# tongdaxu/VQ-VAE-from-Gaussian-VAE

Measured on AMD Instinct MI355X. Metric: images/sec encode+quantize+decode, 256x256, codebook 2^16, higher is better.
Workload: dtype f32

## Files before the change

vq-vae-from-gaussian-vae_amd/csrc/gq_conv3.h:

```cpp
#pragma once
#include <type_traits>

#include "gq_common.h"
#include "gq_epilogue.h"
#include "gq_stats.h"
#include "gq_wino_gemm.h"

namespace gqhip {

constexpr int kC3TH = 8, kC3TW = 32;
constexpr int kC3PH = kC3TH + 2, kC3PW = kC3TW + 2;
constexpr int kC3Pix = kC3PH * kC3PW;
constexpr int kC3RS = 48;
constexpr int kC3Plane = kC3PH * kC3RS * 32;
constexpr int kC3Buf = 2 * kC3Plane;
constexpr int kC3Pieces = kC3Pix * 4;
constexpr int kC3Loads = (kC3Pieces + 255) / 256;

__device__ __forceinline__ int conv3_lds_off(int R, int x, int half) {
  return (R * kC3RS + x) * 32 + 16 * (half ^ ((x >> 3) & 1));
}

struct Conv3Params {
  const _Float16 *Xs;
  const _Float16 *Wf;
  const float *bias;
  const float *res;
  float *y;
  int64_t *stats;
  int H, W, nch, cpg;
  int cout, nnb;
  int tiles_x, tiles_y;
  long ntiles;
  long tiles_per_xcd;
  float mscale;
};

struct Conv3Tile {
  long b;
  int y0, x0, nb;
};
__device__ __forceinline__ bool conv3_tile(const Conv3Params &p, Conv3Tile &t, long vb = blockIdx.x) {
  const long k = vb >> 3;
  t.nb = (int)(k % p.nnb);
  const long tile = (long)(vb & 7) * p.tiles_per_xcd + k / p.nnb;
  if (tile >= p.ntiles) return false;
  const int tx = (int)(tile % p.tiles_x);
  const long t2 = tile / p.tiles_x;
  t.b = t2 / p.tiles_y;
  t.y0 = (int)(t2 % p.tiles_y) * kC3TH;
  t.x0 = tx * kC3TW;
  return true;
}

__device__ __forceinline__ void conv3_tap(const unsigned char *A, int dy, const f16x8 (&bq)[4], f32x16 (&acc)[4][2]) {
#pragma unroll
  for (int rr = 0; rr < 4; ++rr) {
#if defined(GQHIP_ABL) && (GQHIP_ABL & 256)
    const f16x8 ah = *reinterpret_cast<const f16x8 *>(A + dy * kC3RS * 32);
    const f16x8 al = ah;
#else
    const f16x8 ah = *reinterpret_cast<const f16x8 *>(A + (rr + dy) * kC3RS * 32);
    const f16x8 al = *reinterpret_cast<const f16x8 *>(A + (rr + dy) * kC3RS * 32 + kC3Plane);
#endif
#pragma unroll
    for (int j = 0; j < 2; ++j) {
      acc[rr][j] = __builtin_amdgcn_mfma_f32_32x32x16_f16(ah, bq[2 * j], acc[rr][j], 0, 0, 0);
      acc[rr][j] = __builtin_amdgcn_mfma_f32_32x32x16_f16(ah, bq[2 * j + 1], acc[rr][j], 0, 0, 0);
      acc[rr][j] = __builtin_amdgcn_mfma_f32_32x32x16_f16(al, bq[2 * j], acc[rr][j], 0, 0, 0);
    }
  }
}

template <int COUT, int RR>
__device__ __forceinline__ void conv3_epilogue(const Conv3Params &p, const Conv3Tile &t, const f32x16 (&acc)[RR][2], unsigned char *sA,
                                               int64_t *red, int wave, int wm, int wn) {
  constexpr int cout = COUT;
  const int lane = __lane_id(), tid = wave * 64 + lane;
  const int n = wn * 64 + 4 * (lane & 15);
  float *stage = reinterpret_cast<float *>(sA + wave * kEpiWaveBytes);
  f32x4 pb = {0.f, 0.f, 0.f, 0.f};
  if (p.bias) {
#pragma unroll
    for (int e = 0; e < 4; ++e) pb[e] = p.bias[t.nb * 128 + n + e];
  }
  const long o = ((t.b * p.H + t.y0 + RR * wm) * p.W + t.x0 + (lane >> 4)) * cout + t.nb * 128 + n;
  const long slice = (long)p.W * cout;
  StatPartial st;
  if (!p.stats) {
    if (p.res) epi_store<3, false>(acc, stage, lane, p.y, p.res, o, slice, 4 * cout, p.mscale, pb, st);
    else epi_store<2, false>(acc, stage, lane, p.y, nullptr, o, slice, 4 * cout, p.mscale, pb, st);
    return;
  }
  if constexpr (RR == 4) {
    if (p.res) epi_store<3, true>(acc, stage, lane, p.y, p.res, o, slice, 4 * cout, p.mscale, pb, st);
    else epi_store<2, true>(acc, stage, lane, p.y, nullptr, o, slice, 4 * cout, p.mscale, pb, st);
    stat_partial_flush(red + kStatWords * (n / p.cpg), st);
  } else {
    __shared__ double part[2 * 64 * 4];
    double *mine = part + (wn * 64 + lane) * 4;
    if (wm == 0) {
      if (p.res) epi_store<3, true>(acc, stage, lane, p.y, p.res, o, slice, 4 * cout, p.mscale, pb, st);
      else epi_store<2, true>(acc, stage, lane, p.y, nullptr, o, slice, 4 * cout, p.mscale, pb, st);
      mine[0] = st.v0; mine[1] = st.s; mine[2] = st.ss; mine[3] = (double)st.n;
    }
    __syncthreads();
    if (wm == 1) {
      st.v0 = mine[0]; st.s = mine[1]; st.ss = mine[2]; st.n = (int)mine[3];
      if (p.res) epi_store<3, true>(acc, stage, lane, p.y, p.res, o, slice, 4 * cout, p.mscale, pb, st);
      else epi_store<2, true>(acc, stage, lane, p.y, nullptr, o, slice, 4 * cout, p.mscale, pb, st);
      stat_partial_flush(red + kStatWords * (n / p.cpg), st);
    }
  }
  __syncthreads();
  const int gpb = 128 / p.cpg, groups = cout / p.cpg;
  if (tid < kStatWords * gpb) stat_flush_word(p.stats + kStatWords * (t.b * groups + t.nb * gpb) + tid, red[tid]);
}

#define GQ_C3_ZERO_ACC(acc)                                                                                         \
  _Pragma("unroll") for (int rr = 0; rr < 4; ++rr) _Pragma("unroll") for (int j = 0; j < 2; ++j) acc[rr][j] =       \
      f32x16{0.f, 0.f, 0.f, 0.f, 0.f, 0.f, 0.f, 0.f, 0.f, 0.f, 0.f, 0.f, 0.f, 0.f, 0.f, 0.f}

struct Conv3GnParams {
  Conv3Params c;
  const float *x;
  const float *gamma, *beta, *pre_bias;
  const int64_t *stats_in;
  int cin, cpg_in;
  double eps;
  float scale;
};

#ifdef GQHIP_CLOCK_STAMPS
__device__ unsigned long long g_c3_stamps[4 * 8192];
#endif
template <int SILU, int COUT>
__global__ __launch_bounds__(256, 2) void conv3x3_gn_f16x3_kernel(const Conv3GnParams pp) {
  typedef _Float16 f16x4 __attribute__((ext_vector_type(4)));
  const Conv3Params &p = pp.c;
  __shared__ __attribute__((aligned(16))) unsigned char sA[2 * kC3Buf];
  __shared__ int64_t red[kStatWords * 32];
  __shared__ __attribute__((aligned(16))) float sAff[2][512];
  const int tid = threadIdx.x, lane = tid & 63, wave = __builtin_amdgcn_readfirstlane(tid >> 6);
  const int c = lane & 31, h = lane >> 5, wm = wave >> 1, wn = wave & 1;
#ifdef GQHIP_CLOCK_STAMPS
  const unsigned long long st_r0 = __builtin_amdgcn_s_memrealtime();
#endif
  Conv3Tile t;
  if (!conv3_tile(p, t)) return;
  const int H = p.H, W = p.W, cin = pp.cin;
  red[tid] = 0;
  {
    const int groups = cin / pp.cpg_in;
    const double n = (double)pp.cpg_in * (double)H * (double)W;
    for (int ch = tid; ch < cin; ch += 256) {
      const int g = ch / pp.cpg_in;
      double st_s, st_ss;
      stat_load(pp.stats_in + kStatWords * (t.b * groups + g), st_s, st_ss);
      const double mean = st_s / n;
      double var = st_ss / n - mean * mean;
      var = var > 0.0 ? var : 0.0;
      const double rstd = 1.0 / sqrt(var + pp.eps);
      const double pbk = pp.pre_bias ? (double)pp.pre_bias[ch] : 0.0;
      sAff[0][ch] = (float)(rstd * (double)pp.gamma[ch]);
      sAff[1][ch] = (float)((double)pp.beta[ch] + (pbk - mean) * rstd * (double)pp.gamma[ch]);
    }
  }
  const int w = tid & 3, qs = tid >> 2;
  int goff[kC3Loads];
  unsigned inb = 0;
#pragma unroll
  for (int i = 0; i < kC3Loads; ++i) {
    int q = qs + 64 * i;
    q = q < kC3Pix ? q : kC3Pix - 1;
    const int R = q / kC3PW, px = q % kC3PW;
    const int gy = t.y0 - 1 + R, gx = t.x0 - 1 + px;
    const bool in = gy >= 0 && gy < H && gx >= 0 && gx < W;
    const int cy = gy < 0 ? 0 : (gy >= H ? H - 1 : gy), cx = gx < 0 ? 0 : (gx >= W ? W - 1 : gx);
    goff[i] = (cy * W + cx) * cin + 4 * w;
    inb |= (unsigned)(in ? 1 : 0) << i;
  }
  const float *xb = pp.x + t.b * (long)H * W * cin;
  f32x4 st[3];
  auto issue = [&](int i, int chunk) { st[i % 3] = *reinterpret_cast<const f32x4 *>(xb + goff[i] + chunk * 16); };
  auto convert = [&](int i, int chunk, int buf) {
    const int q = qs + 64 * i;
    if (q >= kC3Pix) return;
    const f32x4 a4 = *reinterpret_cast<const f32x4 *>(&sAff[0][chunk * 16 + 4 * w]);
    const f32x4 sh4 = *reinterpret_cast<const f32x4 *>(&sAff[1][chunk * 16 + 4 * w]);
    const f32x4 v = gn_act<SILU>(st[i % 3], a4, sh4) * (((inb >> i) & 1) ? pp.scale : 0.f);
    f16x4 hi, lo;
#pragma unroll
    for (int e = 0; e < 4; ++e) {
      hi[e] = (_Float16)v[e];
      lo[e] = (_Float16)(v[e] - (float)hi[e]);
    }
    const int off = buf * kC3Buf + conv3_lds_off(q / kC3PW, q % kC3PW, w >> 1) + 8 * (w & 1);
    *reinterpret_cast<f16x4 *>(&sA[off]) = hi;
    *reinterpret_cast<f16x4 *>(&sA[off + kC3Plane]) = lo;
  };

  f32x16 acc[4][2];
  GQ_C3_ZERO_ACC(acc);
  int aoff[3];
#pragma unroll
  for (int dx = 0; dx < 3; ++dx) aoff[dx] = conv3_lds_off(4 * wm, c + dx, h);
  const unsigned char *wbase = reinterpret_cast<const unsigned char *>(p.Wf) + (4 * t.nb + 2 * wn) * 128 * 16;
  const int wl = lane * 16;
  const long wstep = (long)p.nnb * (512 * 16);
  f16x8 bs[3][4];
  auto load_b = [&](int ks, f16x8 (&dst)[4]) {
    const unsigned char *s = wbase + ks * wstep;
#pragma unroll
    for (int k = 0; k < 4; ++k) dst[k] = *reinterpret_cast<const f16x8 *>(s + k * 1024 + wl);
  };
  const int nks = p.nch * 9;
// ... 188 lines not shown
      for (int i = 0; i < NI; ++i) convert(i, nbuf);
    }
    __builtin_amdgcn_sched_barrier(0);
    __syncthreads();
  }
  if constexpr (SPLIT != 0) {
    const int C = p.cout / 3, col = t.nb * 128, third = col / C;
    const int n = wn * 64 + 4 * (lane & 15), cc = col - third * C + n;
    const long L = (long)p.H * 32, tok = (long)(t.y0 + RR * wm) * 32 + (lane >> 4);
    f32x4 pb = {0.f, 0.f, 0.f, 0.f};
    if (p.bias) {
#pragma unroll
      for (int e = 0; e < 4; ++e) pb[e] = p.bias[col + n + e];
    }
    float *stage = reinterpret_cast<float *>(sA + wave * kEpiWaveBytes);
    if (third < 2) {
      _Float16 *dst = third == 0 ? pp.Q3 : pp.K3;
      epi_store_split(acc, stage, lane, dst, (t.b * L + tok) * 3 * C + cc, 32L * 3 * C, 4L * 3 * C, (long)C, third == 0, p.mscale,
                      pb, pp.sq);
    } else {
      epi_store_split(acc, stage, lane, pp.V3, (t.b * 3 * L + tok) * C + cc, 32L * C, 4L * C, L * C, false, p.mscale, pb, pp.sv);
    }
  } else {
    conv3_epilogue<COUT>(p, t, acc, sA, red, wave, wm, wn);
  }
}

struct Conv3S2Params {
  Conv3Params c;
  const float *x;
  const float *scales_dev;
  float scale;
  int cin, Hin, Win;
};

template <int COUT>
__global__ __launch_bounds__(256, 2) void conv3x3s2_f16x3_kernel(const Conv3S2Params pp) {
  typedef _Float16 f16x4 __attribute__((ext_vector_type(4)));
  Conv3Params p = pp.c;
  __shared__ __attribute__((aligned(16))) unsigned char sA[2 * kC3Buf];
  __shared__ int64_t red[kStatWords * 32];
  const int tid = threadIdx.x, lane = tid & 63, wave = __builtin_amdgcn_readfirstlane(tid >> 6);
  const int c = lane & 31, h = lane >> 5, wm = wave >> 1, wn = wave & 1;
  Conv3Tile t;
  if (!conv3_tile(p, t)) return;
  red[tid] = 0;
  const float scale = pp.scales_dev ? pp.scales_dev[0] : pp.scale;
  if (pp.scales_dev) p.mscale = pp.scales_dev[1];
  const int cin = pp.cin, nch = p.nch, Hin = pp.Hin, Win = pp.Win;
  constexpr int PR = kC3TH + 1, PC = kC3TW + 1, NP = 5;
  const int w = tid & 3, qs = tid >> 2;
  const float *xb = pp.x + t.b * (long)Hin * Win * cin + 4 * w;
  int goff[NP], loff[NP];
  unsigned inb = 0;
  auto setup_phase = [&](int a, int b) {
    inb = 0;
#pragma unroll
    for (int i = 0; i < NP; ++i) {
      const int q = qs + 64 * i;
      const int qq = q < PR * PC ? q : PR * PC - 1;
      const int R = qq / PC, X = qq % PC;
      const int gy = 2 * (t.y0 + R) + a, gx = 2 * (t.x0 + X) + b;
      const bool in = gy < Hin && gx < Win;
      const int cy = gy < Hin ? gy : Hin - 1, cx = gx < Win ? gx : Win - 1;
      goff[i] = (cy * Win + cx) * cin;
      loff[i] = q < PR * PC ? conv3_lds_off(R, X, w >> 1) + 8 * (w & 1) : -1;
      inb |= (unsigned)(in ? 1 : 0) << i;
    }
  };
  f32x4 st[NP];
  auto issue = [&](int chunk) {
#pragma unroll
    for (int i = 0; i < NP; ++i) st[i] = *reinterpret_cast<const f32x4 *>(xb + goff[i] + chunk * 16);
  };
  auto commit = [&](int buf) {
#pragma unroll
    for (int i = 0; i < NP; ++i) {
      if (loff[i] < 0) continue;
      const f32x4 v = st[i] * (((inb >> i) & 1) ? scale : 0.f);
      f16x4 hi, lo;
#pragma unroll
      for (int e = 0; e < 4; ++e) {
        hi[e] = (_Float16)v[e];
        lo[e] = (_Float16)(v[e] - (float)hi[e]);
      }
      unsigned char *d = sA + buf * kC3Buf + loff[i];
      *reinterpret_cast<f16x4 *>(d) = hi;
      *reinterpret_cast<f16x4 *>(d + kC3Plane) = lo;
    }
  };
  f32x16 acc[4][2];
  GQ_C3_ZERO_ACC(acc);
  int aoff[2];
#pragma unroll
  for (int dx = 0; dx < 2; ++dx) aoff[dx] = conv3_lds_off(4 * wm, c + dx, h);
  const unsigned char *wbase = reinterpret_cast<const unsigned char *>(p.Wf) + (4 * t.nb + 2 * wn) * 128 * 16;
  const int wl = lane * 16;
  const long wstep = (long)p.nnb * (512 * 16);
  f16x8 bq[4], bn[4];
  auto load_b = [&](int ks, f16x8 (&dst)[4]) {
    const unsigned char *s = wbase + ks * wstep;
#pragma unroll
    for (int k = 0; k < 4; ++k) dst[k] = *reinterpret_cast<const f16x8 *>(s + k * 1024 + wl);
  };
  const int nks = 9 * nch;
  int ks = 0, unit = 0;
  load_b(0, bq);
  setup_phase(0, 0);
  issue(0);
  commit(0);
  __syncthreads();
  auto run_unit = [&](auto nt_tag, auto a_tag, auto b_tag, int chunk) {
    constexpr int NT = decltype(nt_tag)::value, PA = decltype(a_tag)::value, PB = decltype(b_tag)::value;
    const bool last_chunk = chunk + 1 >= nch;
    const bool more = !(last_chunk && PA == 1 && PB == 1);
    if (more) {
      if (last_chunk) setup_phase(PB == 1 ? 1 : PA, PB == 1 ? 0 : 1);
      issue(last_chunk ? 0 : chunk + 1);
    }
    const unsigned char *A = sA + (unit & 1) * kC3Buf;
#pragma unroll
    for (int ti = 0; ti < NT; ++ti) {
      const int ddy = (PA == 0 && PB == 0) ? ti / 2 : (PA == 0 && PB == 1) ? ti : 0;
      const int ddx = (PA == 0 && PB == 0) ? ti % 2 : (PA == 1 && PB == 0) ? ti : 0;
      load_b(ks + 1 < nks ? ks + 1 : ks, bn);
      conv3_tap(A + aoff[ddx], ddy, bq, acc);
#pragma unroll
      for (int k = 0; k < 4; ++k) bq[k] = bn[k];
      ++ks;
      __builtin_amdgcn_sched_barrier(0);
    }
    if (more) commit((unit + 1) & 1);
    ++unit;
    __syncthreads();
  };
  using I0 = std::integral_constant<int, 0>; using I1 = std::integral_constant<int, 1>;
  using I2 = std::integral_constant<int, 2>; using I4 = std::integral_constant<int, 4>;
  for (int chunk = 0; chunk < nch; ++chunk) run_unit(I4{}, I0{}, I0{}, chunk);
  for (int chunk = 0; chunk < nch; ++chunk) run_unit(I2{}, I0{}, I1{}, chunk);
  for (int chunk = 0; chunk < nch; ++chunk) run_unit(I2{}, I1{}, I0{}, chunk);
  for (int chunk = 0; chunk < nch; ++chunk) run_unit(I1{}, I1{}, I1{}, chunk);
  conv3_epilogue<COUT>(p, t, acc, sA, red, wave, wm, wn);
}

struct Upconv2Params {
  Conv3Params c;
  const float *x;
  const float *scales_dev;
  float scale;
  int cin;
};

template <int COUT>
__global__ __launch_bounds__(256, 2) void upconv2x_f16x3_kernel(const Upconv2Params pp) {
  typedef _Float16 f16x4 __attribute__((ext_vector_type(4)));
  Conv3Params p = pp.c;
  __shared__ __attribute__((aligned(16))) unsigned char sA[2 * kC3Buf];
  __shared__ int64_t red[kStatWords * 32];
  const int tid = threadIdx.x, lane = tid & 63, wave = __builtin_amdgcn_readfirstlane(tid >> 6);
  const int c = lane & 31, h = lane >> 5, wm = wave >> 1, wn = wave & 1;
  Conv3Tile t;
  if (!conv3_tile(p, t)) return;
  const int pa = (int)blockIdx.y >> 1, pb = (int)blockIdx.y & 1;
  red[tid] = 0;
  const float scale = pp.scales_dev ? pp.scales_dev[0] : pp.scale;
  if (pp.scales_dev) p.mscale = pp.scales_dev[1];
  const int cin = pp.cin, nch = p.nch, H = p.H, W = p.W;
  constexpr int PR = kC3TH + 1, PC = kC3TW + 1, NP = 5;
  const int w = tid & 3, qs = tid >> 2;
  const float *xb = pp.x + t.b * (long)H * W * cin + 4 * w;
  int goff[NP], loff[NP];
  unsigned inb = 0;
#pragma unroll
  for (int i = 0; i < NP; ++i) {
    const int q = qs + 64 * i;
    const int qq = q < PR * PC ? q : PR * PC - 1;
    const int R = qq / PC, X = qq % PC;
    const int gy = t.y0 + R + pa - 1, gx = t.x0 + X + pb - 1;
    const bool in = gy >= 0 && gy < H && gx >= 0 && gx < W;
    const int cy = gy < 0 ? 0 : (gy >= H ? H - 1 : gy), cx = gx < 0 ? 0 : (gx >= W ? W - 1 : gx);
    goff[i] = (cy * W + cx) * cin;
    loff[i] = q < PR * PC ? conv3_lds_off(R, X, w >> 1) + 8 * (w & 1) : -1;
    inb |= (unsigned)(in ? 1 : 0) << i;
  }
  f32x4 st[NP];
  auto issue = [&](int chunk) {
#pragma unroll
    for (int i = 0; i < NP; ++i) st[i] = *reinterpret_cast<const f32x4 *>(xb + goff[i] + chunk * 16);
  };
  auto commit = [&](int buf) {
#pragma unroll
    for (int i = 0; i < NP; ++i) {
      if (loff[i] < 0) continue;
      const f32x4 v = st[i] * (((inb >> i) & 1) ? scale : 0.f);
      f16x4 hi, lo;
#pragma unroll
      for (int e = 0; e < 4; ++e) {
        hi[e] = (_Float16)v[e];
        lo[e] = (_Float16)(v[e] - (float)hi[e]);
      }
      unsigned char *d = sA + buf * kC3Buf + loff[i];
      *reinterpret_cast<f16x4 *>(d) = hi;
      *reinterpret_cast<f16x4 *>(d + kC3Plane) = lo;
    }
  };
  f32x16 acc[4][2];
  GQ_C3_ZERO_ACC(acc);
  int aoff[2];
#pragma unroll
  for (int dx = 0; dx < 2; ++dx) aoff[dx] = conv3_lds_off(4 * wm, c + dx, h);
  const long wstep = (long)p.nnb * (512 * 16);
  const int nks = 4 * nch;
  const unsigned char *wbase = reinterpret_cast<const unsigned char *>(p.Wf) + (long)blockIdx.y * nks * wstep +
                               (4 * t.nb + 2 * wn) * 128 * 16;
  const int wl = lane * 16;
  f16x8 b0[4], b1[4], b2[4];
  auto load_b = [&](int ks, f16x8 (&dst)[4]) {
    const unsigned char *s = wbase + (long)(ks < nks ? ks : nks - 1) * wstep;
#pragma unroll
    for (int k = 0; k < 4; ++k) dst[k] = *reinterpret_cast<const f16x8 *>(s + k * 1024 + wl);
  };
  load_b(0, b0);
  load_b(1, b1);
  issue(0);
  commit(0);
  __syncthreads();
  int ks = 0;
  for (int chunk = 0; chunk < nch; ++chunk) {
    const bool more = chunk + 1 < nch;
    if (more) issue(chunk + 1);
    const unsigned char *A = sA + (chunk & 1) * kC3Buf;
#pragma unroll
    for (int ti = 0; ti < 4; ++ti) {
      load_b(ks + 2, b2);
      conv3_tap(A + aoff[ti & 1], ti >> 1, b0, acc);
#pragma unroll
      for (int k = 0; k < 4; ++k) {
        b0[k] = b1[k];
        b1[k] = b2[k];
      }
      ++ks;
      __builtin_amdgcn_sched_barrier(0);
    }
    if (more) commit((chunk + 1) & 1);
    __syncthreads();
  }
  constexpr int cout = COUT;
  const int n = wn * 64 + 4 * (lane & 15);
  f32x4 bias4 = {0.f, 0.f, 0.f, 0.f};
  if (p.bias) {
#pragma unroll
    for (int e = 0; e < 4; ++e) bias4[e] = p.bias[t.nb * 128 + n + e];
  }
  float *stage = reinterpret_cast<float *>(sA + wave * kEpiWaveBytes);
  const long W2 = 2L * W;
  const long o = ((t.b * 2L * H + 2 * (t.y0 + 4 * wm) + pa) * W2 + 2 * (t.x0 + (lane >> 4)) + pb) * cout + t.nb * 128 + n;
  StatPartial sp;
  if (!p.stats) {
    epi_store<1, false>(acc, stage, lane, p.y, nullptr, o, 2 * W2 * cout, 8 * cout, p.mscale, bias4, sp);
    return;
  }
  epi_store<1, true>(acc, stage, lane, p.y, nullptr, o, 2 * W2 * cout, 8 * cout, p.mscale, bias4, sp);
  stat_partial_flush(red + kStatWords * (n / p.cpg), sp);
  __syncthreads();
  const int gpb = 128 / p.cpg, groups = cout / p.cpg;
  if (tid < kStatWords * gpb) stat_flush_word(p.stats + kStatWords * (t.b * groups + t.nb * gpb) + tid, red[tid]);
}

template <int SILU, int COUT>
__global__ __launch_bounds__(256) void conv3x3_gn_small_kernel(const float *__restrict__ x, const float *__restrict__ gamma,
                                                               const float *__restrict__ beta,
                                                               const float *__restrict__ pre_bias,
                                                               const int64_t *__restrict__ stats, const float *__restrict__ w,
                                                               const float *__restrict__ bias, float *__restrict__ y, int H,
                                                               int W, int C, int cpg, double eps) {
  constexpr int PW = 18, PS = 36;
  __shared__ __attribute__((aligned(16))) float sX[PW * PW * PS];
  __shared__ __attribute__((aligned(16))) float sAff[2][512];
  const int tid = threadIdx.x, tx = tid & 15, ty = tid >> 4;
  const int tiles_x = W / 16, tiles_y = H / 16;
  const int txb = blockIdx.x % tiles_x, tyb = (blockIdx.x / tiles_x) % tiles_y;
  const long b = blockIdx.x / (tiles_x * tiles_y);
  const int y0 = tyb * 16, x0 = txb * 16;
  {
    const int groups = C / cpg;
    const double n = (double)cpg * (double)H * (double)W;
    for (int ch = tid; ch < C; ch += 256) {
      const int g = ch / cpg;
      double st_s, st_ss;
      stat_load(stats + kStatWords * (b * groups + g), st_s, st_ss);
      const double mean = st_s / n;
      double var = st_ss / n - mean * mean;
      var = var > 0.0 ? var : 0.0;
      const double rstd = 1.0 / sqrt(var + eps);
      const double pbk = pre_bias ? (double)pre_bias[ch] : 0.0;
      sAff[0][ch] = (float)(rstd * (double)gamma[ch]);
      sAff[1][ch] = (float)((double)beta[ch] + (pbk - mean) * rstd * (double)gamma[ch]);
    }
  }
  float acc[COUT];
#pragma unroll
  for (int co = 0; co < COUT; ++co) acc[co] = bias ? bias[co] : 0.f;
  const float *xb = x + b * (long)H * W * C;
  __syncthreads();
  for (int c0 = 0; c0 < C; c0 += 32) {
    for (int i = tid; i < PW * PW * 8; i += 256) {
      const int px = i >> 3, q = i & 7;
      const int R = px / PW, X = px % PW;
      const int gy = y0 - 1 + R, gx = x0 - 1 + X;
      const bool in = gy >= 0 && gy < H && gx >= 0 && gx < W;
      const int cy = gy < 0 ? 0 : (gy >= H ? H - 1 : gy), cx = gx < 0 ? 0 : (gx >= W ? W - 1 : gx);
      const f32x4 v = *reinterpret_cast<const f32x4 *>(xb + ((long)cy * W + cx) * C + c0 + 4 * q);
      const f32x4 a4 = *reinterpret_cast<const f32x4 *>(&sAff[0][c0 + 4 * q]);
      const f32x4 sh4 = *reinterpret_cast<const f32x4 *>(&sAff[1][c0 + 4 * q]);
      *reinterpret_cast<f32x4 *>(&sX[px * PS + 4 * q]) = gn_act<SILU>(v, a4, sh4) * (in ? 1.f : 0.f);
    }
    __syncthreads();
#pragma unroll
    for (int tap = 0; tap < 9; ++tap) {
      const float *s = &sX[((ty + tap / 3) * PW + tx + tap % 3) * PS];
#pragma unroll
      for (int q = 0; q < 8; ++q) {
        const f32x4 v = *reinterpret_cast<const f32x4 *>(s + 4 * q);
#pragma unroll
        for (int co = 0; co < COUT; ++co) {
          const float *wp = w + ((long)(co * 9 + tap) * C + c0 + 4 * q);
          acc[co] = __builtin_fmaf(v.x, wp[0], acc[co]);
          acc[co] = __builtin_fmaf(v.y, wp[1], acc[co]);
          acc[co] = __builtin_fmaf(v.z, wp[2], acc[co]);
          acc[co] = __builtin_fmaf(v.w, wp[3], acc[co]);
        }
      }
    }
    __syncthreads();
  }
  float *yo = y + ((b * H + y0 + ty) * W + x0 + tx) * COUT;
#pragma unroll
  for (int co = 0; co < COUT; ++co) yo[co] = acc[co];
}

}
```

vq-vae-from-gaussian-vae_amd/csrc/gqhip_unet.hip:

```cpp
#include "gqhip.h"

#include <hip/hip_ext.h>
#include <hip/hip_runtime.h>

#include <cstdlib>
#include <cstring>

#include "gqhip_internal.h"
#include "gq_unet_aux.h"
#include "gq_wino_gemm.h"
#include "gq_conv3.h"
#include "gq_conv_f32.h"
#include "gq_attn.h"

using namespace gqhip;

namespace {
thread_local int g_stats_prezeroed = 0;
inline hipError_t stats_zero(void *p, size_t bytes, hipStream_t st) {
  return g_stats_prezeroed ? hipSuccess : hipMemsetAsync(p, 0, bytes, st);
}
}

extern "C" {
// ... 286 lines not shown
  conv3_fill(cp, Wf, bias_or_null, res_or_null, y, stats_out_or_null, B, H, W, Cin, Cout, groups_out, mscale);
  gp.x = x; gp.gamma = gamma; gp.beta = beta; gp.pre_bias = pre_bias_or_null; gp.stats_in = stats_in;
  gp.cin = (int)Cin; gp.cpg_in = (int)(Cin / groups_in); gp.eps = eps; gp.scale = scale;
  const dim3 grid((unsigned)(8 * cp.tiles_per_xcd * cp.nnb));
  static const int env_dyn = getenv("GQHIP_C3_DYNLDS") ? atoi(getenv("GQHIP_C3_DYNLDS")) : 0;
  if (Cout == 128) {
    if (apply_silu) hipLaunchKernelGGL((conv3x3_gn_f16x3_kernel<1, 128>), grid, dim3(256), env_dyn, st, gp);
    else hipLaunchKernelGGL((conv3x3_gn_f16x3_kernel<0, 128>), grid, dim3(256), 0, st, gp);
  } else {
    if (apply_silu) hipLaunchKernelGGL((conv3x3_gn_f16x3_kernel<1, 256>), grid, dim3(256), 0, st, gp);
    else hipLaunchKernelGGL((conv3x3_gn_f16x3_kernel<0, 256>), grid, dim3(256), 0, st, gp);
  }
  return check_launch();
}

#ifdef GQHIP_CLOCK_STAMPS
extern "C" int gqhip_debug_c3_stamps(unsigned long long *out, int64_t words) {
  return hipMemcpyFromSymbol(out, HIP_SYMBOL(g_c3_stamps), sizeof(unsigned long long) * words) == hipSuccess ? 0 : 1;
}
#endif

static int conv1_tile_rows(int64_t B, int64_t HW, int64_t Cout) {
  const char *knob = getenv("GQHIP_CONV1_TILE");
  if (knob && !strcmp(knob, "128")) return 2;
  if (knob && !strcmp(knob, "256")) return HW % 256 == 0 ? 4 : 0;
  if (HW % 256 != 0) return 2;
  static thread_local int cus_of[64];
  int dev = 0;
  if (hipGetDevice(&dev) != hipSuccess || dev < 0 || dev >= 64) return 4;
  if (cus_of[dev] == 0) {
    int n = 0;
    if (hipDeviceGetAttribute(&n, hipDeviceAttributeMultiprocessorCount, dev) != hipSuccess || n < 1) return 4;
    cus_of[dev] = n;
  }
  const int64_t slots = 2 * (int64_t)cus_of[dev], blocks = B * (HW / 256) * (Cout / 128);
  if (blocks < slots) return 2;
  const int64_t last = blocks % slots;
  return (last != 0 && last * 100 < slots * 85) ? 2 : 4;
}

#define GQ_C1_LAUNCH(RR, GN)                                                                                             \
  do {                                                                                                                   \
    if (split) hipLaunchKernelGGL((conv1x1_f16x3_kernel<0, RR, GN, 1>), grid, dim3(256), 0, st, gp);                     \
    else if (Cout == 128) hipLaunchKernelGGL((conv1x1_f16x3_kernel<128, RR, GN, 0>), grid, dim3(256), 0, st, gp);        \
    else if (Cout == 256) hipLaunchKernelGGL((conv1x1_f16x3_kernel<256, RR, GN, 0>), grid, dim3(256), 0, st, gp);        \
    else if (Cout == 512) hipLaunchKernelGGL((conv1x1_f16x3_kernel<512, RR, GN, 0>), grid, dim3(256), 0, st, gp);        \
    else hipLaunchKernelGGL((conv1x1_f16x3_kernel<1536, RR, GN, 0>), grid, dim3(256), 0, st, gp);                        \
  } while (0)

static int conv1_launch(Conv1Params &gp, const void *Wf, float mscale, const float *bias, const float *res, float *y,
                        int64_t *stats_out, int64_t B, int64_t HW, int64_t Cin, int64_t Cout, int64_t groups_out, void *stream) {
  const bool split = gp.Q3 != nullptr, gn = gp.gamma != nullptr;
  const int rows = conv1_tile_rows(B, HW, Cout);
  if (rows == 0) return GQHIP_ERR_INVALID_ARG;
  hipStream_t st = static_cast<hipStream_t>(stream);
  if (stats_out && stats_zero(stats_out, sizeof(int64_t) * kStatWords * B * groups_out, st) != hipSuccess) return check_launch();
  Conv3Params &cp = gp.c;
  conv3_fill(cp, Wf, bias, res, y, stats_out, B, HW / 32, 32, Cin, Cout, groups_out, mscale);
  cp.nch = (int)(Cin / 16);
  cp.tiles_x = 1; cp.tiles_y = (int)(HW / (64 * rows));
  cp.ntiles = (long)B * cp.tiles_y;
  cp.tiles_per_xcd = (cp.ntiles + 7) / 8;
  gp.cin = (int)Cin;
  const dim3 grid((unsigned)(8 * cp.tiles_per_xcd * cp.nnb));
  if (rows == 4) {
    if (gn) GQ_C1_LAUNCH(4, 1); else GQ_C1_LAUNCH(4, 0);
  } else {
    if (gn) GQ_C1_LAUNCH(2, 1); else GQ_C1_LAUNCH(2, 0);
  }
#undef GQ_C1_LAUNCH
  return check_launch();
}

static bool conv1_shape_ok(int64_t B, int64_t HW, int64_t Cin) {
  return B >= 0 && HW >= 128 && HW % 128 == 0 && Cin >= 32 && Cin % 32 == 0 && HW <= (1 << 24);
}

static bool conv1_gn_ok(int64_t Cin, int64_t groups_in) {
  return Cin <= 512 && groups_in >= 1 && Cin % groups_in == 0 && (Cin / groups_in) % 4 == 0;
}

int conv1x1_f16x3(const float *x, const float *pre_bias_or_null, const void *Wf, const float *scales_dev_or_null, float scale,
                  float mscale, const float *bias_or_null, const float *res_or_null, float *y, int64_t *stats_out_or_null, int64_t B, int64_t HW,
                  int64_t Cin, int64_t Cout, int64_t groups_out, void *stream) {
  if (!conv1_shape_ok(B, HW, Cin) || (Cout != 128 && Cout != 256 && Cout != 512 && Cout != 1536) ||
      (!scales_dev_or_null && !(scale > 0.f)))
    return GQHIP_ERR_INVALID_ARG;
  if (stats_out_or_null && !conv3_groups_ok(Cout, groups_out)) return GQHIP_ERR_INVALID_ARG;
  if (B == 0) return GQHIP_OK;
  if (!x || !Wf || !y) return GQHIP_ERR_INVALID_ARG;
  Conv1Params gp{};
  gp.x = x; gp.pre_bias = pre_bias_or_null; gp.scales_dev = scales_dev_or_null; gp.scale = scale;
  return conv1_launch(gp, Wf, mscale, bias_or_null, res_or_null, y, stats_out_or_null, B, HW, Cin, Cout, groups_out, stream);
}

int conv1x1_gn_f16x3(const float *x, const float *gamma, const float *beta, const float *pre_bias_or_null,
                     const int64_t *stats_in, int64_t groups_in, double eps, const void *Wf, float scale, float mscale,
                     const float *bias_or_null, const float *res_or_null, float *y, int64_t *stats_out_or_null, int64_t B,
                     int64_t HW, int64_t Cin, int64_t Cout, int64_t groups_out, void *stream) {
  if (!conv1_shape_ok(B, HW, Cin) || !conv1_gn_ok(Cin, groups_in) || (Cout != 128 && Cout != 256 && Cout != 512 && Cout != 1536) ||
      !(scale > 0.f))
    return GQHIP_ERR_INVALID_ARG;
  if (stats_out_or_null && !conv3_groups_ok(Cout, groups_out)) return GQHIP_ERR_INVALID_ARG;
  if (B == 0) return GQHIP_OK;
  if (!x || !gamma || !beta || !stats_in || !Wf || !y) return GQHIP_ERR_INVALID_ARG;
  Conv1Params gp{};
  gp.x = x; gp.pre_bias = pre_bias_or_null; gp.scale = scale;
  gp.gamma = gamma; gp.beta = beta; gp.stats_in = stats_in; gp.cpg_in = (int)(Cin / groups_in); gp.eps = eps;
  return conv1_launch(gp, Wf, mscale, bias_or_null, res_or_null, y, stats_out_or_null, B, HW, Cin, Cout, groups_out, stream);
}

int conv1x1_qkv_split_f16x3(const float *x, const float *gamma_or_null, const float *beta_or_null, const float *pre_bias_or_null,
                            const int64_t *stats_in_or_null, int64_t groups_in, double eps, const void *Wf, float scale,
                            float mscale, const float *bias_or_null, void *Q3, void *K3, void *V3, float sq, float sv, int64_t B,
                            int64_t L, int64_t C, void *stream) {
  if (!conv1_shape_ok(B, L, C) || C % 128 != 0 || !(scale > 0.f) || !(sq > 0.f) || !(sv > 0.f))
    return GQHIP_ERR_INVALID_ARG;
  if (gamma_or_null && !conv1_gn_ok(C, groups_in)) return GQHIP_ERR_INVALID_ARG;
  if (B == 0) return GQHIP_OK;
  if (!x || !Wf || !Q3 || !K3 || !V3 || (gamma_or_null && (!beta_or_null || !stats_in_or_null))) return GQHIP_ERR_INVALID_ARG;
  Conv1Params gp{};
  gp.x = x; gp.pre_bias = pre_bias_or_null; gp.scale = scale;
  if (gamma_or_null) {
    gp.gamma = gamma_or_null; gp.beta = beta_or_null; gp.stats_in = stats_in_or_null; gp.cpg_in = (int)(C / groups_in); gp.eps = eps;
  }
  gp.Q3 = static_cast<_Float16 *>(Q3); gp.K3 = static_cast<_Float16 *>(K3); gp.V3 = static_cast<_Float16 *>(V3);
  gp.sq = sq; gp.sv = sv;
  return conv1_launch(gp, Wf, mscale, bias_or_null, nullptr, nullptr, nullptr, B, L, C, 3 * C, 1, stream);
}

int conv3x3s2_f16x3(const float *x, const void *Wf, const float *scales_dev_or_null, float scale, float mscale,
                    const float *bias_or_null, float *y, int64_t *stats_out_or_null, int64_t B, int64_t Hin, int64_t Win,
                    int64_t Cin, int64_t Cout, int64_t groups_out, void *stream) {
  if (B < 0 || Hin < 2 * kC3TH || Win < 2 * kC3TW || Hin % (2 * kC3TH) || Win % (2 * kC3TW) || Cin < 16 || Cin % 16 != 0 ||
      (Cout != 128 && Cout != 256 && Cout != 512) || Hin * Win > (1 << 24) || (!scales_dev_or_null && !(scale > 0.f)))
    return GQHIP_ERR_INVALID_ARG;
  if (stats_out_or_null && !conv3_groups_ok(Cout, groups_out)) return GQHIP_ERR_INVALID_ARG;
  if (B == 0) return GQHIP_OK;
  if (!x || !Wf || !y) return GQHIP_ERR_INVALID_ARG;
  hipStream_t st = static_cast<hipStream_t>(stream);
  if (stats_out_or_null && stats_zero(stats_out_or_null, sizeof(int64_t) * kStatWords * B * groups_out, st) != hipSuccess)
    return check_launch();
  Conv3S2Params gp{};
  Conv3Params &cp = gp.c;
  conv3_fill(cp, Wf, bias_or_null, nullptr, y, stats_out_or_null, B, Hin / 2, Win / 2, Cin, Cout, groups_out, mscale);
  gp.x = x; gp.scales_dev = scales_dev_or_null; gp.scale = scale; gp.cin = (int)Cin; gp.Hin = (int)Hin; gp.Win = (int)Win;
  const dim3 grid((unsigned)(8 * cp.tiles_per_xcd * cp.nnb));
  if (Cout == 128) hipLaunchKernelGGL(conv3x3s2_f16x3_kernel<128>, grid, dim3(256), 0, st, gp);
  else if (Cout == 256) hipLaunchKernelGGL(conv3x3s2_f16x3_kernel<256>, grid, dim3(256), 0, st, gp);
  else hipLaunchKernelGGL(conv3x3s2_f16x3_kernel<512>, grid, dim3(256), 0, st, gp);
  return check_launch();
}

int upconv2x_f16x3(const float *x, const void *Wf, const float *scales_dev_or_null, float scale, float mscale,
                   const float *bias_or_null, float *y, int64_t *stats_out_or_null, int64_t B, int64_t H, int64_t W,
                   int64_t Cin, int64_t Cout, int64_t groups_out, void *stream) {
  if (B < 0 || H < kC3TH || W < kC3TW || H % kC3TH || W % kC3TW || Cin < 16 || Cin % 16 != 0 ||
      (Cout != 128 && Cout != 256 && Cout != 512) || H * W > (1 << 22) || (!scales_dev_or_null && !(scale > 0.f)))
    return GQHIP_ERR_INVALID_ARG;
  if (stats_out_or_null && !conv3_groups_ok(Cout, groups_out)) return GQHIP_ERR_INVALID_ARG;
  if (B == 0) return GQHIP_OK;
  if (!x || !Wf || !y) return GQHIP_ERR_INVALID_ARG;
  hipStream_t st = static_cast<hipStream_t>(stream);
  if (stats_out_or_null && stats_zero(stats_out_or_null, sizeof(int64_t) * kStatWords * B * groups_out, st) != hipSuccess)
    return check_launch();
  Upconv2Params gp{};
  Conv3Params &cp = gp.c;
  conv3_fill(cp, Wf, bias_or_null, nullptr, y, stats_out_or_null, B, H, W, Cin, Cout, groups_out, mscale);
  gp.x = x; gp.scales_dev = scales_dev_or_null; gp.scale = scale; gp.cin = (int)Cin;
  const dim3 grid((unsigned)(8 * cp.tiles_per_xcd * cp.nnb), 4);
  if (Cout == 128) hipLaunchKernelGGL(upconv2x_f16x3_kernel<128>, grid, dim3(256), 0, st, gp);
  else if (Cout == 256) hipLaunchKernelGGL(upconv2x_f16x3_kernel<256>, grid, dim3(256), 0, st, gp);
  else hipLaunchKernelGGL(upconv2x_f16x3_kernel<512>, grid, dim3(256), 0, st, gp);
  return check_launch();
}

int conv3x3_gn_small_f32(const float *x, const float *gamma, const float *beta, const float *pre_bias_or_null,
                         const int64_t *stats_in, int64_t groups_in, double eps, int apply_silu, const float *w_ohwi,
                         const float *bias_or_null, float *y, int64_t B, int64_t H, int64_t W, int64_t Cin, int64_t Cout,
                         void *stream) {
  if (B < 0 || H < 16 || W < 16 || H % 16 || W % 16 || Cin < 32 || Cin % 32 != 0 || Cin > 512 || Cout < 1 || Cout > 4 ||
      groups_in < 1 || Cin % groups_in != 0 || B * (H / 16) * (W / 16) > 0x7fffffffL)
    return GQHIP_ERR_INVALID_ARG;
  if (B == 0) return GQHIP_OK;
  if (!x || !gamma || !beta || !stats_in || !w_ohwi || !y) return GQHIP_ERR_INVALID_ARG;
  hipStream_t st = static_cast<hipStream_t>(stream);
  const dim3 grid((unsigned)(B * (H / 16) * (W / 16)));
  const int cpg = (int)(Cin / groups_in);
#define GQ_CS(S, CO)                                                                                                      \
  hipLaunchKernelGGL((conv3x3_gn_small_kernel<S, CO>), grid, dim3(256), 0, st, x, gamma, beta, pre_bias_or_null, stats_in, \
                     w_ohwi, bias_or_null, y, (int)H, (int)W, (int)Cin, cpg, eps)
#define GQ_CS2(CO) do { if (apply_silu) GQ_CS(1, CO); else GQ_CS(0, CO); } while (0)
  switch (Cout) {
    case 1: GQ_CS2(1); break;
    case 2: GQ_CS2(2); break;
    case 3: GQ_CS2(3); break;
    default: GQ_CS2(4); break;
  }
#undef GQ_CS2
#undef GQ_CS
  return check_launch();
}

int conv3x3_cin_small_f32(const float *x, const float *wk, const float *bias_or_null, float *y, int64_t *stats_out_or_null,
                          int64_t B, int64_t H, int64_t W, int64_t Cin, int64_t Cout, int64_t groups_out, void *stream) {
  if (B < 0 || H < 8 || W < 32 || H % 8 || W % 32 || Cin < 1 || Cin > 4 || Cout != 128 || B * (H / 8) * (W / 32) > 0x7fffffffL)
    return GQHIP_ERR_INVALID_ARG;
  if (stats_out_or_null && groups_out != 32) return GQHIP_ERR_INVALID_ARG;
  if (B == 0) return GQHIP_OK;
  if (!x || !wk || !y) return GQHIP_ERR_INVALID_ARG;
  hipStream_t st = static_cast<hipStream_t>(stream);
  if (stats_out_or_null && stats_zero(stats_out_or_null, sizeof(int64_t) * kStatWords * B * 32, st) != hipSuccess)
    return check_launch();
  ConvInParams cp{};
  cp.x = x; cp.wk = wk; cp.bias = bias_or_null; cp.y = y; cp.stats = stats_out_or_null; cp.H = (int)H; cp.W = (int)W;
  const dim3 grid((unsigned)(B * (H / 8) * (W / 32)));
  switch (Cin) {
    case 1: hipLaunchKernelGGL(conv3x3_cin_small_kernel<1>, grid, dim3(256), 0, st, cp); break;
    case 2: hipLaunchKernelGGL(conv3x3_cin_small_kernel<2>, grid, dim3(256), 0, st, cp); break;
    case 3: hipLaunchKernelGGL(conv3x3_cin_small_kernel<3>, grid, dim3(256), 0, st, cp); break;
    default: hipLaunchKernelGGL(conv3x3_cin_small_kernel<4>, grid, dim3(256), 0, st, cp); break;
  }
  return check_launch();
}

int conv3x3_f32(const float *x, const float *gamma_or_null, const float *beta_or_null, const float *pre_bias_or_null,
                const int64_t *stats_or_null, int64_t groups_in, double eps, int apply_silu, const float *wk,
                const float *bias_or_null, float *y, int64_t B, int64_t H, int64_t W, int64_t Cin, int64_t Cout, void *stream) {
  if (B < 0 || H < 1 || W < 1 || Cin < 8 || Cout < 4 || Cout % 4 != 0 || B * H * ((W + 31) / 32) > 0x7fffffffL)
    return GQHIP_ERR_INVALID_ARG;
  if (B == 0) return GQHIP_OK;
  if (!x || !wk || !y) return GQHIP_ERR_INVALID_ARG;
  const bool gn = stats_or_null != nullptr;
  if (gn && (!gamma_or_null || !beta_or_null || groups_in < 1 || Cin % groups_in != 0 || Cin > 1024)) return GQHIP_ERR_INVALID_ARG;
  hipStream_t st = static_cast<hipStream_t>(stream);
  ConvF32Params cp{};
  cp.x = x; cp.gamma = gamma_or_null; cp.beta = beta_or_null; cp.pre_bias = pre_bias_or_null; cp.stats = stats_or_null;
  cp.wk = wk; cp.bias = bias_or_null; cp.y = y;
  cp.H = (int)H; cp.W = (int)W; cp.Cin = (int)Cin; cp.Cout = (int)Cout; cp.cpg = gn ? (int)(Cin / groups_in) : 1; cp.eps = eps;
  const unsigned segs = (unsigned)(B * H * ((W + 31) / 32));
  if (Cin % 64 == 0) {
    const dim3 grid(segs, (unsigned)((Cout + 31) / 32));
    if (gn && apply_silu) hipLaunchKernelGGL((conv3x3_f32_ksplit_kernel<true, 1>), grid, dim3(256), 0, st, cp);
    else if (gn) hipLaunchKernelGGL((conv3x3_f32_ksplit_kernel<true, 0>), grid, dim3(256), 0, st, cp);
    else hipLaunchKernelGGL((conv3x3_f32_ksplit_kernel<false, 0>), grid, dim3(256), 0, st, cp);
    return check_launch();
  }
  if (gn) return GQHIP_ERR_INVALID_ARG;
  switch (Cin) {
    case 8: hipLaunchKernelGGL((conv3x3_f32_nsplit_kernel<8>), dim3(segs), dim3(256), 0, st, cp); break;
    case 16: hipLaunchKernelGGL((conv3x3_f32_nsplit_kernel<16>), dim3(segs), dim3(256), 0, st, cp); break;
    case 32: hipLaunchKernelGGL((conv3x3_f32_nsplit_kernel<32>), dim3(segs), dim3(256), 0, st, cp); break;
    default: return GQHIP_ERR_INVALID_ARG;
  }
  return check_launch();
}

int wino_out_nhwc_f32(const float *M, float *y, int64_t B, int64_t H, int64_t W, int64_t C, float mscale, void *stream) {
  if (B < 0 || H < 2 || W < 2 || H % 2 || W % 2 || C < 4 || C % 4 != 0) return GQHIP_ERR_INVALID_ARG;
  if (B == 0) return GQHIP_OK;
  if (!M || !y) return GQHIP_ERR_INVALID_ARG;
  const long tiles = (long)(B * (H / 2) * (W / 2)), total = tiles * (C / 4);
  long blocks = (total + 255) / 256;
  if (blocks > 16384) blocks = 16384;
  return launch(wino_out_nhwc_kernel, dim3((unsigned)blocks), dim3(256), 0, static_cast<hipStream_t>(stream), M, y,
                (int)H, (int)W, (int)(C / 4), tiles, total, mscale);
}

int wino4_in_nhwc_f32(const float *x, float *V, int64_t B, int64_t H, int64_t W, int64_t C, void *stream) {
  if (B < 0 || H < 4 || W < 4 || H % 4 || W % 4 || C < 4 || C % 4 != 0) return GQHIP_ERR_INVALID_ARG;
  if (B == 0) return GQHIP_OK;
  if (!x || !V) return GQHIP_ERR_INVALID_ARG;
  const long tiles = (long)(B * (H / 4) * (W / 4)), total = tiles * (C / 4);
  long blocks = (total + 255) / 256;
  if (blocks > 16384) blocks = 16384;
  return launch(wino4_in_nhwc_kernel<0>, dim3((unsigned)blocks), dim3(256), 0, static_cast<hipStream_t>(stream), x,
                (void *)V, (int)H, (int)W, (int)(C / 4), tiles, total, 1.0f);
}

int wino4_out_nhwc_f32(const float *M, float *y, int64_t B, int64_t H, int64_t W, int64_t C, float mscale, void *stream) {
  if (B < 0 || H < 4 || W < 4 || H % 4 || W % 4 || C < 4 || C % 4 != 0) return GQHIP_ERR_INVALID_ARG;
  if (B == 0) return GQHIP_OK;
  if (!M || !y) return GQHIP_ERR_INVALID_ARG;
  const long tiles = (long)(B * (H / 4) * (W / 4)), total = tiles * (C / 4);
  long blocks = (total + 255) / 256;
  if (blocks > 16384) blocks = 16384;
  return launch(wino4_out_nhwc_kernel, dim3((unsigned)blocks), dim3(256), 0, static_cast<hipStream_t>(stream), M, y,
                (int)H, (int)W, (int)(C / 4), tiles, total, mscale);
}

int wino_out_res_nhwc_f32(const float *M, const float *res, const float *bias_or_null, float *y, int64_t *stats_out,
                          int64_t B, int64_t H, int64_t W, int64_t C, int64_t groups, int tile, float mscale,
                          void *stream) {
  if ((tile != 2 && tile != 4) || B < 0 || H < tile || W < tile || H % tile || W % tile || C < 4 || C % 4 != 0 ||
      groups < 1 || C % groups != 0)
    return GQHIP_ERR_INVALID_ARG;
  if (B == 0) return GQHIP_OK;
  if (!M || !y || !stats_out) return GQHIP_ERR_INVALID_ARG;
  const int64_t cpg = C / groups;
  if (cpg % 4 != 0 || 256 % (C / 4) != 0 || groups > 64) return GQHIP_ERR_INVALID_ARG;
  hipStream_t st = static_cast<hipStream_t>(stream);
  if (stats_zero(stats_out, sizeof(int64_t) * kStatWords * B * groups, st) != hipSuccess) return check_launch();
  const long tpi = (long)((H / tile) * (W / tile)), tiles = (long)B * tpi;
  const int vw = (tile == 4 && 256 % (C / 2) == 0) ? 2 : 4;
  const int lanes = (int)(256 / (C / vw));
  long slabs = (tpi + (long)lanes * 4 - 1) / ((long)lanes * 4);
  if (slabs > 1024) slabs = 1024;
  if (slabs < 1) slabs = 1;
  const dim3 grid((unsigned)(B * slabs));
  if (tile == 4 && vw == 2)
    hipLaunchKernelGGL((wino_out_res_nhwc_kernel<4, 2>), grid, dim3(256), 0, st, M, res, bias_or_null, y, stats_out, (int)H,
                       (int)W, (int)(C / 2), (int)cpg, tiles, (int)slabs, mscale);
  else if (tile == 4)
    hipLaunchKernelGGL((wino_out_res_nhwc_kernel<4, 4>), grid, dim3(256), 0, st, M, res, bias_or_null, y, stats_out, (int)H,
                       (int)W, (int)(C / 4), (int)cpg, tiles, (int)slabs, mscale);
  else
    hipLaunchKernelGGL((wino_out_res_nhwc_kernel<2, 4>), grid, dim3(256), 0, st, M, res, bias_or_null, y, stats_out, (int)H,
                       (int)W, (int)(C / 4), (int)cpg, tiles, (int)slabs, mscale);
  return check_launch();
}

int attn_split_qkv_f16x3(const float *qkv, void *Q3, void *K3, void *V3, int64_t B, int64_t L, int64_t C, float sq, float sv,
                         void *stream) {
  if (B < 0 || L < 1 || C < 4 || C % 4 != 0 || !(sq > 0.f) || !(sv > 0.f)) return GQHIP_ERR_INVALID_ARG;
  if (B == 0) return GQHIP_OK;
  if (!qkv || !Q3 || !K3 || !V3) return GQHIP_ERR_INVALID_ARG;
// ... 72 lines not shown
```

Measured before the change: 507.3.

## Add 4-row upconv tile computing both column phases per block with software-pipelined staging

Adds a new default upconv kernel path that uses 4 low-resolution rows per block. Each block's waves cover both column phases (pb) for one row phase (pa), so the staged input halo tile is shared across two output phases instead of being loaded once per phase. The next chunk's global loads and f32-to-f16 hi/lo conversions are spread between the MFMA taps to overlap them. The shorter tile also shrinks LDS per block. In exchange the halo overhead per output grows and the launch grid changes. An env var keeps the old 8-row path available.

Result: no change. 509.5, median of 6 (+0.4%).

```diff
diff --git a/vq-vae-from-gaussian-vae_amd/csrc/gq_conv3.h b/vq-vae-from-gaussian-vae_amd/csrc/gq_conv3.h
--- a/vq-vae-from-gaussian-vae_amd/csrc/gq_conv3.h
+++ b/vq-vae-from-gaussian-vae_amd/csrc/gq_conv3.h
@@ -4,6 +4,7 @@
 #include "gq_common.h"
 #include "gq_epilogue.h"
 #include "gq_stats.h"
+#include "gq_upconv_tile.h"
 #include "gq_wino_gemm.h"
 
 namespace gqhip {
@@ -53,6 +54,7 @@
   return true;
 }
 
+template <int PLANE = kC3Plane>
 __device__ __forceinline__ void conv3_tap(const unsigned char *A, int dy, const f16x8 (&bq)[4], f32x16 (&acc)[4][2]) {
 #pragma unroll
   for (int rr = 0; rr < 4; ++rr) {
@@ -61,7 +63,7 @@
     const f16x8 al = ah;
 #else
     const f16x8 ah = *reinterpret_cast<const f16x8 *>(A + (rr + dy) * kC3RS * 32);
-    const f16x8 al = *reinterpret_cast<const f16x8 *>(A + (rr + dy) * kC3RS * 32 + kC3Plane);
+    const f16x8 al = *reinterpret_cast<const f16x8 *>(A + (rr + dy) * kC3RS * 32 + PLANE);
 #endif
 #pragma unroll
     for (int j = 0; j < 2; ++j) {
@@ -556,7 +558,33 @@
 };
 
 template <int COUT>
-__global__ __launch_bounds__(256, 2) void upconv2x_f16x3_kernel(const Upconv2Params pp) {
+__device__ __forceinline__ void upconv_epilogue(const Conv3Params &p, long b, int row0, int x0, int nb, int pa, int pb,
+                                                const f32x16 (&acc)[4][2], unsigned char *sA, int64_t *red, int wave, int wn) {
+  constexpr int cout = COUT;
+  const int lane = __lane_id(), tid = wave * 64 + lane;
+  const int n = wn * 64 + 4 * (lane & 15);
+  f32x4 bias4 = {0.f, 0.f, 0.f, 0.f};
+  if (p.bias) {
+#pragma unroll
+    for (int e = 0; e < 4; ++e) bias4[e] = p.bias[nb * 128 + n + e];
+  }
+  float *stage = reinterpret_cast<float *>(sA + wave * kEpiWaveBytes);
+  const long W2 = 2L * p.W;
+  const long o = ((b * 2L * p.H + 2 * row0 + pa) * W2 + 2 * (x0 + (lane >> 4)) + pb) * cout + nb * 128 + n;
+  StatPartial sp;
+  if (!p.stats) {
+    epi_store<1, false>(acc, stage, lane, p.y, nullptr, o, 2 * W2 * cout, 8 * cout, p.mscale, bias4, sp);
+    return;
+  }
+  epi_store<1, true>(acc, stage, lane, p.y, nullptr, o, 2 * W2 * cout, 8 * cout, p.mscale, bias4, sp);
+  stat_partial_flush(red + kStatWords * (n / p.cpg), sp);
+  __syncthreads();
+  const int gpb = 128 / p.cpg, groups = cout / p.cpg;
+  if (tid < kStatWords * gpb) stat_flush_word(p.stats + kStatWords * (b * groups + nb * gpb) + tid, red[tid]);
+}
+
+template <int COUT>
+__device__ __forceinline__ void upconv2x_one_phase(const Upconv2Params &pp) {
   typedef _Float16 f16x4 __attribute__((ext_vector_type(4)));
   Conv3Params p = pp.c;
   __shared__ __attribute__((aligned(16))) unsigned char sA[2 * kC3Buf];
@@ -649,26 +677,116 @@
     if (more) commit((chunk + 1) & 1);
     __syncthreads();
   }
-  constexpr int cout = COUT;
-  const int n = wn * 64 + 4 * (lane & 15);
-  f32x4 bias4 = {0.f, 0.f, 0.f, 0.f};
-  if (p.bias) {
-#pragma unroll
-    for (int e = 0; e < 4; ++e) bias4[e] = p.bias[t.nb * 128 + n + e];
-  }
-  float *stage = reinterpret_cast<float *>(sA + wave * kEpiWaveBytes);
-  const long W2 = 2L * W;
-  const long o = ((t.b * 2L * H + 2 * (t.y0 + 4 * wm) + pa) * W2 + 2 * (t.x0 + (lane >> 4)) + pb) * cout + t.nb * 128 + n;
-  StatPartial sp;
-  if (!p.stats) {
-    epi_store<1, false>(acc, stage, lane, p.y, nullptr, o, 2 * W2 * cout, 8 * cout, p.mscale, bias4, sp);
-    return;
-  }
-  epi_store<1, true>(acc, stage, lane, p.y, nullptr, o, 2 * W2 * cout, 8 * cout, p.mscale, bias4, sp);
-  stat_partial_flush(red + kStatWords * (n / p.cpg), sp);
+  upconv_epilogue<COUT>(p, t.b, t.y0 + 4 * wm, t.x0, t.nb, pa, pb, acc, sA, red, wave, wn);
+}
+
+constexpr int kU4PH = 5, kU4PW = kC3TW + 2, kU4Pix = kU4PH * kU4PW;
+constexpr int kU4Plane = kU4PH * kC3RS * 32;
+constexpr int kU4Buf = 2 * kU4Plane;
+constexpr int kU4NP = (kU4Pix * 4 + 255) / 256;
+constexpr int kU4LDS = 2 * kU4Buf > 4 * kEpiWaveBytes ? 2 * kU4Buf : 4 * kEpiWaveBytes;
+
+template <int COUT>
+__device__ __forceinline__ void upconv2x_two_phase(const Upconv2Params &pp) {
+  typedef _Float16 f16x4 __attribute__((ext_vector_type(4)));
+  static_assert(kU4NP == 3, "one conversion after each of taps 1, 2, 3");
+  Conv3Params p = pp.c;
+  __shared__ __attribute__((aligned(16))) unsigned char sA[kU4LDS];
+  __shared__ int64_t red[kStatWords * 32];
+  const int tid = threadIdx.x, lane = tid & 63, wave = __builtin_amdgcn_readfirstlane(tid >> 6);
+  const int c = lane & 31, h = lane >> 5, pb = wave >> 1, wn = wave & 1;
+  UpconvTile t;
+  if (!upconv_tile4((long)blockIdx.x, p.nnb, p.tiles_x, p.tiles_y, p.ntiles, p.tiles_per_xcd, t)) return;
+  const int pa = t.pa, y0 = 4 * t.ty, x0 = kC3TW * t.tx;
+  red[tid] = 0;
+  const float scale = pp.scales_dev ? pp.scales_dev[0] : pp.scale;
+  if (pp.scales_dev) p.mscale = pp.scales_dev[1];
+  const int cin = pp.cin, nch = p.nch, H = p.H, W = p.W;
+  const int w = tid & 3, qs = tid >> 2;
+  const float *xb = pp.x + t.b * (long)H * W * cin + 4 * w;
+  int goff[kU4NP], loff[kU4NP];
+  unsigned inb = 0;
+#pragma unroll
+  for (int i = 0; i < kU4NP; ++i) {
+    const int q = qs + 64 * i;
+    const int qq = q < kU4Pix ? q : kU4Pix - 1;
+    const int R = qq / kU4PW, X = qq % kU4PW;
+    const int gy = y0 + R + pa - 1, gx = x0 + X - 1;
+    const bool in = gy >= 0 && gy < H && gx >= 0 && gx < W;
+    const int cy = gy < 0 ? 0 : (gy >= H ? H - 1 : gy), cx = gx < 0 ? 0 : (gx >= W ? W - 1 : gx);
+    goff[i] = (cy * W + cx) * cin;
+    loff[i] = q < kU4Pix ? conv3_lds_off(R, X, w >> 1) + 8 * (w & 1) : -1;
+    inb |= (unsigned)(in ? 1 : 0) << i;
+  }
+  f32x4 st[kU4NP];
+  auto issue = [&](int chunk) {
+#pragma unroll
+    for (int i = 0; i < kU4NP; ++i) st[i] = *reinterpret_cast<const f32x4 *>(xb + goff[i] + chunk * 16);
+  };
+  auto convert = [&](int i, int buf) {
+    if (loff[i] < 0) return;
+    const f32x4 v = st[i] * (((inb >> i) & 1) ? scale : 0.f);
+    f16x4 hi, lo;
+#pragma unroll
+    for (int e = 0; e < 4; ++e) {
+      hi[e] = (_Float16)v[e];
+      lo[e] = (_Float16)(v[e] - (float)hi[e]);
+    }
+    unsigned char *d = sA + buf * kU4Buf + loff[i];
+    *reinterpret_cast<f16x4 *>(d) = hi;
+    *reinterpret_cast<f16x4 *>(d + kU4Plane) = lo;
+  };
+  f32x16 acc[4][2];
+  GQ_C3_ZERO_ACC(acc);
+  int aoff[2];
+#pragma unroll
+  for (int v = 0; v < 2; ++v) aoff[v] = conv3_lds_off(0, c + pb + v, h);
+  const long wstep = (long)p.nnb * (512 * 16);
+  const int nks = 4 * nch;
+  const unsigned char *wbase = reinterpret_cast<const unsigned char *>(p.Wf) + (long)(2 * pa + pb) * nks * wstep +
+                               (4 * t.nb + 2 * wn) * 128 * 16;
+  const int wl = lane * 16;
+  f16x8 b0[4], b1[4], b2[4];
+  auto load_b = [&](int ks, f16x8 (&dst)[4]) {
+    const unsigned char *s = wbase + (long)(ks < nks ? ks : nks - 1) * wstep;
+#pragma unroll
+    for (int k = 0; k < 4; ++k) dst[k] = *reinterpret_cast<const f16x8 *>(s + k * 1024 + wl);
+  };
+  load_b(0, b0);
+  load_b(1, b1);
+  issue(0);
+#pragma unroll
+  for (int i = 0; i < kU4NP; ++i) convert(i, 0);
   __syncthreads();
-  const int gpb = 128 / p.cpg, groups = cout / p.cpg;
-  if (tid < kStatWords * gpb) stat_flush_word(p.stats + kStatWords * (t.b * groups + t.nb * gpb) + tid, red[tid]);
+  int ks = 0;
+  for (int chunk = 0; chunk < nch; ++chunk) {
+    const bool more = chunk + 1 < nch;
+    const unsigned char *A = sA + (chunk & 1) * kU4Buf;
+    const int nbuf = (chunk + 1) & 1;
+#pragma unroll
+    for (int ti = 0; ti < 4; ++ti) {
+      load_b(ks + 2, b2);
+      conv3_tap<kU4Plane>(A + aoff[ti & 1], ti >> 1, b0, acc);
+#pragma unroll
+      for (int k = 0; k < 4; ++k) {
+        b0[k] = b1[k];
+        b1[k] = b2[k];
+      }
+      ++ks;
+      if (ti == 0) issue(more ? chunk + 1 : chunk);
+      else if (more) convert(ti - 1, nbuf);
+      __builtin_amdgcn_sched_barrier(0);
+    }
+    __syncthreads();
+  }
+  upconv_epilogue<COUT>(p, t.b, y0, x0, t.nb, pa, pb, acc, sA, red, wave, wn);
+}
+
+template <int COUT, int TH>
+__global__ __launch_bounds__(256, 2) void upconv2x_f16x3_kernel(const Upconv2Params pp) {
+  static_assert(TH == 8 || TH == 4, "low-resolution rows per block");
+  if constexpr (TH == 8) upconv2x_one_phase<COUT>(pp);
+  else upconv2x_two_phase<COUT>(pp);
 }
 
 template <int SILU, int COUT>
diff --git a/vq-vae-from-gaussian-vae_amd/csrc/gq_upconv_tile.h b/vq-vae-from-gaussian-vae_amd/csrc/gq_upconv_tile.h
--- /dev/null
+++ b/vq-vae-from-gaussian-vae_amd/csrc/gq_upconv_tile.h
@@ -0,0 +1,32 @@
+#pragma once
+
+#if defined(__HIPCC__)
+#define GQ_UPT_FN __host__ __device__ __forceinline__
+#else
+#define GQ_UPT_FN inline
+#endif
+
+namespace gqhip {
+
+struct UpconvTile {
+  long b;
+  int ty, tx;
+  int nb, pa;
+};
+
+GQ_UPT_FN bool upconv_tile4(long vb, int nnb, int tiles_x, int tiles_y, long ntiles, long tiles_per_xcd, UpconvTile &t) {
+  const long k = vb >> 3;
+  const long per_tile = 2L * nnb;
+  const int r = (int)(k % per_tile);
+  const long tile = (vb & 7) * tiles_per_xcd + k / per_tile;
+  if (tile >= ntiles) return false;
+  t.nb = r % nnb;
+  t.pa = r / nnb;
+  t.tx = (int)(tile % tiles_x);
+  const long t2 = tile / tiles_x;
+  t.ty = (int)(t2 % tiles_y);
+  t.b = t2 / tiles_y;
+  return true;
+}
+
+}
diff --git a/vq-vae-from-gaussian-vae_amd/csrc/gqhip_unet.hip b/vq-vae-from-gaussian-vae_amd/csrc/gqhip_unet.hip
--- a/vq-vae-from-gaussian-vae_amd/csrc/gqhip_unet.hip
+++ b/vq-vae-from-gaussian-vae_amd/csrc/gqhip_unet.hip
@@ -462,6 +462,11 @@
   return check_launch();
 }
 
+static int upconv_tile_rows() {
+  const char *knob = getenv("GQHIP_UPCONV_TILE");
+  return knob && !strcmp(knob, "8") ? 8 : 4;
+}
+
 int upconv2x_f16x3(const float *x, const void *Wf, const float *scales_dev_or_null, float scale, float mscale,
                    const float *bias_or_null, float *y, int64_t *stats_out_or_null, int64_t B, int64_t H, int64_t W,
                    int64_t Cin, int64_t Cout, int64_t groups_out, void *stream) {
@@ -471,6 +476,8 @@
   if (stats_out_or_null && !conv3_groups_ok(Cout, groups_out)) return GQHIP_ERR_INVALID_ARG;
   if (B == 0) return GQHIP_OK;
   if (!x || !Wf || !y) return GQHIP_ERR_INVALID_ARG;
+  const int rows = upconv_tile_rows();
+  if (rows == 4 && B * (H / 4) * (W / kC3TW) > (0x7fffffffL - 8) / 16) return GQHIP_ERR_INVALID_ARG;
   hipStream_t st = static_cast<hipStream_t>(stream);
   if (stats_out_or_null && stats_zero(stats_out_or_null, sizeof(int64_t) * kStatWords * B * groups_out, st) != hipSuccess)
     return check_launch();
@@ -478,10 +485,23 @@
   Conv3Params &cp = gp.c;
   conv3_fill(cp, Wf, bias_or_null, nullptr, y, stats_out_or_null, B, H, W, Cin, Cout, groups_out, mscale);
   gp.x = x; gp.scales_dev = scales_dev_or_null; gp.scale = scale; gp.cin = (int)Cin;
-  const dim3 grid((unsigned)(8 * cp.tiles_per_xcd * cp.nnb), 4);
-  if (Cout == 128) hipLaunchKernelGGL(upconv2x_f16x3_kernel<128>, grid, dim3(256), 0, st, gp);
-  else if (Cout == 256) hipLaunchKernelGGL(upconv2x_f16x3_kernel<256>, grid, dim3(256), 0, st, gp);
-  else hipLaunchKernelGGL(upconv2x_f16x3_kernel<512>, grid, dim3(256), 0, st, gp);
+#define GQ_UP_LAUNCH(TH)                                                                                    \
+  do {                                                                                                      \
+    if (Cout == 128) hipLaunchKernelGGL((upconv2x_f16x3_kernel<128, TH>), grid, dim3(256), 0, st, gp);      \
+    else if (Cout == 256) hipLaunchKernelGGL((upconv2x_f16x3_kernel<256, TH>), grid, dim3(256), 0, st, gp); \
+    else hipLaunchKernelGGL((upconv2x_f16x3_kernel<512, TH>), grid, dim3(256), 0, st, gp);                  \
+  } while (0)
+  if (rows == 4) {
+    cp.tiles_y = (int)(H / 4);
+    cp.ntiles = (long)B * cp.tiles_x * cp.tiles_y;
+    cp.tiles_per_xcd = (cp.ntiles + 7) / 8;
+    const dim3 grid((unsigned)(8 * cp.tiles_per_xcd * 2 * cp.nnb));
+    GQ_UP_LAUNCH(4);
+  } else {
+    const dim3 grid((unsigned)(8 * cp.tiles_per_xcd * cp.nnb), 4);
+    GQ_UP_LAUNCH(8);
+  }
+#undef GQ_UP_LAUNCH
   return check_launch();
 }
 
```
